# tahmidawal/Superresolution_for_PDEs

Hardware: AMD Instinct MI355X
Metric: 20->40 SR training samples/sec at batch 1024 per GPU (fwd+MSE bwd+clip+AdamW) (higher is better)
Workload: dtype f32 (h3: fp32 products from power-of-two-scaled 2-piece fp16 splits on fp16 MFMA, fp32 accumulate); 1 GPU; UNet 20->40 train step, fp32, batch 1024/GPU, 40x40; global_batch=1024, per_gpu_batch=1024, hw=40x40, parallelism=dp1

## Files before the change

superresolution_for_pdes_amd/csrc/conv.hip:

```cpp
#include "conv_common.h"

namespace srpde {



constexpr int BK = 16;
constexpr int LDK = BK + 4;


template <int BM, int BN, int WM, int WN>
__global__ __launch_bounds__(256) void conv_igemm_fwd_kernel(ConvParams p) {
  constexpr int TM = BM / WM, TN = BN / WN, TI = TM / 32, TJ = TN / 32;
  constexpr int A_LOADS = BM / 64;
  constexpr int B_ROWS_PER_PASS = 64;
  constexpr int B_LOADS = BN >= 64 ? BN / 64 : 1;
  extern __shared__ __attribute__((aligned(16))) float smem[];
  float* As = smem;
  float* Bs = smem + 2 * BM * LDK;

  const int tid = threadIdx.x, lane = tid & 63, wave = tid >> 6;
  const int wmi = wave % WM, wni = wave / WM;
  const int nbn = (p.Cout + BN - 1) / BN;
  const int nbm = (p.P + BM - 1) / BM;
  const int wg = xcd_remap(blockIdx.x, nbm * nbn);
// ... 758 lines not shown
    for (int g = 0; g < GA; ++g) {
      const unsigned off = (pok && a_ok[g]) ? (unsigned)(pix * p.lddy * 4 + a_colb[g]) : OOB;
      dma16(rsy, off, lds_addr_of(abase + g * GSTR));
    }
    char* bbase = abase + GA * GSTR;
#pragma unroll
    for (int g = 0; g < GB; ++g) {
      const int iy = yy + b_dy[g], ix = xx + b_dx[g];
      const bool ok = pok && b_ok[g] && iy >= 0 && iy < p.H && ix >= 0 && ix < p.W;
      const int ld = b_second[g] ? ld1 : p.ldx0;
      const unsigned off = ok ? (unsigned)((pix + b_sh[g]) * ld * 4 + b_chb[g]) : OOB;
      dma16(b_second[g] ? rs1 : rs0, off, lds_addr_of(bbase + g * GSTR));
    }
  };

  floatx16 acc[QA][QB], part[QA][QB];
#pragma unroll
  for (int i = 0; i < QA; ++i)
#pragma unroll
    for (int j = 0; j < QB; ++j)
#pragma unroll
      for (int r = 0; r < 16; ++r) acc[i][j][r] = 0.f;

  const int lr = lane & 31, lh = lane >> 5;
  const int wm0 = wmi * TM, wn0 = wni * TN;
  const int ma = wm0 + QA * lr, nb = wn0 + QB * lr;
  const int a_rd = (ma >> 5) * GSTR + (ma & 31) * 4 + lh * 128;
  const int b_rd = GA * GSTR + (nb >> 5) * GSTR + (nb & 31) * 4 + lh * 128;

  const int nsteps = (pend - pbeg + BKW - 1) / BKW;
  if (nsteps > 0) issue(pbeg, 0);
  asm volatile("s_waitcnt vmcnt(0)" ::: "memory");
  __syncthreads();
  for (int s = 0; s < nsteps; ++s) {
    const int buf = s & 1;
    if (s + 1 < nsteps) issue(pbeg + (s + 1) * BKW, buf ^ 1);
    const char* st = lds + buf * STAGE;
    const bool fresh = (s % HP) == 0;
#pragma unroll
    for (int kp = 0; kp < BKW / 2; ++kp) {
      const va_t av = *reinterpret_cast<const va_t*>(st + a_rd + kp * 256);
      const vb_t bv = *reinterpret_cast<const vb_t*>(st + b_rd + kp * 256);
#pragma unroll
      for (int i = 0; i < QA; ++i)
#pragma unroll
        for (int j = 0; j < QB; ++j) {
          const floatx16 c0 = (kp == 0 && fresh) ? floatx16{} : part[i][j];
          part[i][j] = __builtin_amdgcn_mfma_f32_32x32x2f32(vget(av, i), vget(bv, j), c0, 0, 0, 0);
        }
    }
    if ((s + 1) % HP == 0 || s + 1 == nsteps) {
#pragma unroll
      for (int i = 0; i < QA; ++i)
#pragma unroll
        for (int j = 0; j < QB; ++j) acc[i][j] += part[i][j];
    }
    asm volatile("s_waitcnt vmcnt(0)" ::: "memory");
    __syncthreads();
  }

  float* out = p.part + (size_t)split * p.Cout * p.K;
  const int n = n0 + nb;
  if (n < p.K) {
#pragma unroll
    for (int i = 0; i < QA; ++i)
#pragma unroll
      for (int r = 0; r < 16; ++r) {
        const int rc = (r & 3) + 8 * (r >> 2) + 4 * lh;
        const int m = m0 + wm0 + QA * rc + i;
        if (m < p.Cout) {
          float* dst = out + (size_t)m * p.K + n;
          if constexpr (QB == 1) {
            dst[0] = acc[i][0][r];
          } else if constexpr (QB == 2) {
            *reinterpret_cast<float2*>(dst) = make_float2(acc[i][0][r], acc[i][1][r]);
          } else {
            *reinterpret_cast<float4*>(dst) = make_float4(acc[i][0][r], acc[i][1][r], acc[i][2][r], acc[i][3][r]);
          }
        }
      }
  }
}

template <int G>
__global__ void slab_group_sum_kernel(float* __restrict__ part, int splits, long long total) {
  const long long i = (long long)blockIdx.x * blockDim.x + threadIdx.x;
  const long long ngroups = (splits + G - 1) / G;
  if (i >= total * ngroups) return;
  const long long g = i / total, e = i - g * total;
  const int q0 = (int)(g * G), q1 = min(splits, q0 + G);
  float s = 0.f;
  if (q1 - q0 == G) {
    float v[G];
#pragma unroll
    for (int u = 0; u < G; ++u) v[u] = part[(size_t)(q0 + u) * total + e];
#pragma unroll
    for (int u = 0; u < G; ++u) s += v[u];
  } else {
    for (int q = q0; q < q1; ++q) s += part[(size_t)q * total + e];
  }
  part[(size_t)q0 * total + e] = s;
}

__global__ void wgrad_reduce_kernel(const float* __restrict__ part, float* __restrict__ dw, int splits,
                                    int cout, int cin, int cin_real, int taps, int accumulate, int stride) {
  __shared__ float red[4][64];
  const long long K = (long long)taps * cin;
  const long long total = (long long)cout * K;
  const int el = threadIdx.x & 63, grp = threadIdx.x >> 6;
  const long long e = (long long)blockIdx.x * 64 + el;
  float s = 0.f;
  if (e < total) {
    const size_t qs = (size_t)stride * cout * K;
    int q = grp;
    for (; q + 28 < splits; q += 32) {
      float v[8];
#pragma unroll
      for (int u = 0; u < 8; ++u) v[u] = part[(size_t)(q + 4 * u) * qs + e];
#pragma unroll
      for (int u = 0; u < 8; ++u) s += v[u];
    }
    for (; q < splits; q += 4) s += part[(size_t)q * qs + e];
  }
  red[grp][el] = s;
  __syncthreads();
  if (grp == 0 && e < total) {
    const float v = (red[0][el] + red[1][el]) + (red[2][el] + red[3][el]);
    const int n = (int)(e / K);
    const int k = (int)(e - (long long)n * K);
    const int t = k / cin, c = k - t * cin;
    if (c < cin_real) {
      const long long dst = ((long long)n * cin_real + c) * taps + t;
      dw[dst] = accumulate ? dw[dst] + v : v;
    }
  }
}

int wgrad_reduce(const float* part, float* dw, int splits, int cout, int cin, int cin_real, int taps, int accumulate,
                 hipStream_t stream) {
  const long long total = (long long)cout * taps * cin;
  const int blocks = (int)((total + 63) / 64);
  int stride = 1;
  if (total < 65536 && splits >= 128) {
    constexpr int G = 32;
    const long long work = total * ((splits + G - 1) / G);
    hipLaunchKernelGGL(slab_group_sum_kernel<G>, dim3((int)((work + 255) / 256)), dim3(256), 0, stream,
                       const_cast<float*>(part), splits, total);
    SRPDE_LAUNCH_CHECK("srpde_conv_wgrad(reduce groups)");
    stride = G;
    splits = (splits + G - 1) / G;
  }
  hipLaunchKernelGGL(wgrad_reduce_kernel, dim3(blocks), dim3(256), 0, stream, part, dw, splits, cout, cin, cin_real,
                     taps, accumulate, stride);
  SRPDE_LAUNCH_CHECK("srpde_conv_wgrad(reduce)");
  return 0;
}

__global__ void pack_weights_kernel(const float* __restrict__ w, float* __restrict__ wf, float* __restrict__ wd,
                                    int cout, int cin, int cin_real, int taps) {
  const long long total = (long long)cout * taps * cin;
  for (long long e = blockIdx.x * (long long)blockDim.x + threadIdx.x; e < total;
       e += (long long)gridDim.x * blockDim.x) {
    const int c = (int)(e % cin);
    const long long r = e / cin;
    const int t = (int)(r % taps);
    const int n = (int)(r / taps);
    const float v = c < cin_real ? w[((long long)n * cin_real + c) * taps + t] : 0.f;
    if (wf) wf[e] = v;
    if (wd) wd[((long long)c * taps + t) * cout + n] = v;
  }
}

template <int BM, int BN, int WM, int WN>
static int launch_fwd(const ConvParams& p, hipStream_t st) {
  const int nbm = ceil_div(p.P, BM), nbn = ceil_div(p.Cout, BN);
  const size_t lds = (size_t)2 * (BM + BN) * LDK * sizeof(float);
  hipLaunchKernelGGL((conv_igemm_fwd_kernel<BM, BN, WM, WN>), dim3(nbm * nbn), dim3(256), lds, st, p);
  SRPDE_LAUNCH_CHECK("srpde_conv_fwd");
  return 0;
}


template <int BM, int BN, int WM, int WN, int HP>
static int launch_fwd_v2(ConvParams p, hipStream_t st, void* ws, size_t ws_bytes) {
  const int nbm = ceil_div(p.P, BM), nbn = ceil_div(p.Cout, BN);
  const int T = nbm * nbn;
  const size_t lds = (size_t)2 * (BM + BN) * ROW2;
  static int slots = [&] {
    int per_cu = 0, dev = 0, cus = 0;
    (void)hipGetDevice(&dev);
    (void)hipDeviceGetAttribute(&cus, hipDeviceAttributeMultiprocessorCount, dev);
    (void)hipOccupancyMaxActiveBlocksPerMultiprocessor(&per_cu, conv_fwd_v2_kernel<BM, BN, WM, WN, HP>, 256, lds);
    return std::max(1, per_cu) * std::max(1, cus);
  }();
  plan_tail(p, T, slots, BM, BN, ws, ws_bytes);
  const int grid = T - p.ntail + p.ntail * p.tsplit;
  hipLaunchKernelGGL((conv_fwd_v2_kernel<BM, BN, WM, WN, HP>), dim3(grid), dim3(256), lds, st, p);
  SRPDE_LAUNCH_CHECK("srpde_conv_fwd(v2)");
  if (p.ntail > 0) {
    hipLaunchKernelGGL((conv_tail_fixup_kernel<BM, BN>), dim3(p.ntail), dim3(1024), 0, st, p);
    SRPDE_LAUNCH_CHECK("srpde_conv_fwd(tail fixup)");
  }
  return 0;
}


static bool v2_ok(const ConvParams& p) {
  const long long maxld = std::max(p.ldx0, p.c1 ? p.ldx1 : 0);
  return p.c0 % 32 == 0 && p.c1 % 32 == 0 && (long long)p.P * maxld * 4 < (1LL << 31) &&
         (long long)p.Cout * p.K * 4 < (1LL << 31);
}

static int fwd_config(int cout) { return cout % 128 == 0 ? 0 : (cout % 64 == 0 ? 1 : 2); }
static int fwd_bm(int cfg) { return cfg == 0 ? 128 : 256; }

template <int BM, int BN, int WM, int WN>
static int launch_wgrad(const WgradParams& p, hipStream_t st, const WgradBn* bn = nullptr) {
  const int nb = ceil_div(p.Cout, BM) * ceil_div(p.K, BN) * p.splits;
  const size_t lds = (size_t)2 * BKP * ((BM + 4) + (BN + 4)) * sizeof(float);
  if (bn != nullptr)
    hipLaunchKernelGGL((conv_wgrad_kernel<BM, BN, WM, WN, true>), dim3(nb), dim3(256), lds, st, p, *bn);
  else
    hipLaunchKernelGGL((conv_wgrad_kernel<BM, BN, WM, WN, false>), dim3(nb), dim3(256), lds, st, p, WgradBn{});
  SRPDE_LAUNCH_CHECK("srpde_conv_wgrad");
  return 0;
}

template <int BM, int BN, int WM, int WN>
static int launch_wgrad_v2(const WgradParams& p, hipStream_t st) {
  const int nb = ceil_div(p.Cout, BM) * ceil_div(p.K, BN) * p.splits;
  const size_t lds = (size_t)2 * (BM / 32 + BN / 32) * GSTR;
  hipLaunchKernelGGL((conv_wgrad_v2_kernel<BM, BN, WM, WN, 2>), dim3(nb), dim3(256), lds, st, p);
  SRPDE_LAUNCH_CHECK("srpde_conv_wgrad(v2)");
  return 0;
}

// ... 181 lines not shown
```

superresolution_for_pdes_amd/csrc/pointwise.hip:

```cpp
#include "common.h"
#include "resample.h"

namespace srpde {

__global__ void nchw_to_nhwc_kernel(const float* __restrict__ x, float* __restrict__ out, int N, int Cin, int HW,
                                    int Cpad) {
  const long long total = (long long)N * HW;
  for (long long e = blockIdx.x * (long long)blockDim.x + threadIdx.x; e < total;
       e += (long long)gridDim.x * blockDim.x) {
    const long long n = e / HW;
    const int p = (int)(e - n * HW);
    float* o = out + e * Cpad;
    for (int c = 0; c < Cpad; ++c) o[c] = c < Cin ? x[(n * Cin + c) * HW + p] : 0.f;
  }
}

__global__ void nhwc_to_nchw_kernel(const float* __restrict__ x, int ldx, float* __restrict__ out, int N, int C,
                                    int HW) {
  const long long total = (long long)N * C * HW;
  for (long long e = blockIdx.x * (long long)blockDim.x + threadIdx.x; e < total;
       e += (long long)gridDim.x * blockDim.x) {
    const long long nc = e / HW;
    const int p = (int)(e - nc * HW);
    const long long n = nc / C;
// ... 817 lines not shown
    const float4 g = *reinterpret_cast<const float4*>(dm + n * C + c);
    const float s = sa[p];
    float4 o;
    o.x = (d.x * s) * a.x + g.x; o.y = (d.y * s) * a.y + g.y;
    o.z = (d.z * s) * a.z + g.z; o.w = (d.w * s) * a.w + g.w;
    float* dst = dx + p * lddx + c;
    if (accumulate) {
      const float4 old = *reinterpret_cast<const float4*>(dst);
      o.x += old.x; o.y += old.y; o.z += old.z; o.w += old.w;
    }
    *reinterpret_cast<float4*>(dst) = o;
  }
}

__global__ void att_bwd_gating_kernel(const float* __restrict__ dsa_pre, const float* __restrict__ wg,
                                      float* __restrict__ dg, int lddg, long long P, int G, int accumulate) {
  const int G4 = G >> 2;
  const long long total = P * G4;
  for (long long e = blockIdx.x * (long long)blockDim.x + threadIdx.x; e < total;
       e += (long long)gridDim.x * blockDim.x) {
    const long long p = e / G4;
    const int c = (int)(e - p * G4) * 4;
    const float s = dsa_pre[p];
    const float4 w = *reinterpret_cast<const float4*>(wg + c);
    float4 o = make_float4(s * w.x, s * w.y, s * w.z, s * w.w);
    float* dst = dg + p * lddg + c;
    if (accumulate) {
      const float4 old = *reinterpret_cast<const float4*>(dst);
      o.x += old.x; o.y += old.y; o.z += old.z; o.w += old.w;
    }
    *reinterpret_cast<float4*>(dst) = o;
  }
}

__global__ __launch_bounds__(256) void weighted_colsum_kernel(const float* __restrict__ v, int ldv,
                                                              const float* __restrict__ s, long long P, int C,
                                                              int rows_per_blk, float2* __restrict__ part) {
  extern __shared__ float4 red4[];
  const int C4 = C >> 2;
  const int c4 = threadIdx.x % C4, r0 = threadIdx.x / C4, rs = blockDim.x / C4;
  const int active = C4 * rs;
  float4 acc = make_float4(0.f, 0.f, 0.f, 0.f);
  float sacc = 0.f;
  const long long pb = (long long)blockIdx.x * rows_per_blk;
  const long long pe = min(P, pb + rows_per_blk);
  if ((int)threadIdx.x < active) {
    auto row = [&](const float4& a, float w) {
      acc.x += a.x * w; acc.y += a.y * w; acc.z += a.z * w; acc.w += a.w * w;
      if (c4 == 0) sacc += w;
    };
    long long p = pb + r0;
    for (; p + 3 * rs < pe; p += 4 * rs) {
      float4 a[4];
      float w[4];
#pragma unroll
      for (int u = 0; u < 4; ++u) {
        a[u] = *reinterpret_cast<const float4*>(v + (p + u * rs) * ldv + c4 * 4);
        w[u] = s[p + u * rs];
      }
#pragma unroll
      for (int u = 0; u < 4; ++u) row(a[u], w[u]);
    }
    for (; p < pe; p += rs) row(*reinterpret_cast<const float4*>(v + p * ldv + c4 * 4), s[p]);
  }
  red4[threadIdx.x] = acc;
  red4[256 + threadIdx.x] = make_float4(sacc, 0.f, 0.f, 0.f);
  __syncthreads();
  if ((int)threadIdx.x < C4) {
    float4 t = make_float4(0.f, 0.f, 0.f, 0.f);
    float ts = 0.f;
    for (int r = 0; r < rs; ++r) {
      const float4 a = red4[r * C4 + threadIdx.x];
      t.x += a.x; t.y += a.y; t.z += a.z; t.w += a.w;
      if (threadIdx.x == 0) ts += red4[256 + r * C4].x;
    }
    float2* o = part + (size_t)blockIdx.x * (C + 1);
    const int c = threadIdx.x * 4;
    o[c] = make_float2(t.x, 0.f); o[c + 1] = make_float2(t.y, 0.f);
    o[c + 2] = make_float2(t.z, 0.f); o[c + 3] = make_float2(t.w, 0.f);
    if (threadIdx.x == 0) o[C] = make_float2(ts, 0.f);
  }
}

__global__ __launch_bounds__(1024) void outer_sum_kernel(const float* __restrict__ a, int la,
                                                         const float* __restrict__ b, int lb, int n,
                                                         float* __restrict__ out) {
  __shared__ double red[16][64];
  const int i = blockIdx.x, jl = threadIdx.x & 63, grp = threadIdx.x >> 6;
  const int j = blockIdx.y * 64 + jl;
  double s = 0.0;
  if (j < lb) {
    int k = grp;
    for (; k + 7 * 16 < n; k += 8 * 16) {
      float av[8], bv[8];
#pragma unroll
      for (int u = 0; u < 8; ++u) {
        av[u] = a ? a[(long long)(k + 16 * u) * la + i] : 1.f;
        bv[u] = b ? b[(long long)(k + 16 * u) * lb + j] : 1.f;
      }
#pragma unroll
      for (int u = 0; u < 8; ++u) s += (double)av[u] * (double)bv[u];
    }
    for (; k < n; k += 16) {
      const double av = a ? (double)a[(long long)k * la + i] : 1.0;
      const double bv = b ? (double)b[(long long)k * lb + j] : 1.0;
      s += av * bv;
    }
  }
  red[grp][jl] = s;
  __syncthreads();
  if (grp == 0 && j < lb) {
    double t = 0.0;
    for (int g = 0; g < 16; ++g) t += red[g][jl];
    out[(long long)i * lb + j] = (float)t;
  }
}

__global__ void rowsum_kernel(const float* __restrict__ rows, int n, int len, float* __restrict__ out, int stride_in,
                              int accumulate) {
  const int j = blockIdx.x * blockDim.x + threadIdx.x;
  if (j >= len) return;
  double s = 0.0;
  for (int k = 0; k < n; ++k) s += rows[(long long)k * stride_in + j];
  out[j] = accumulate ? out[j] + (float)s : (float)s;
}

__global__ void partsum_kernel(const float2* __restrict__ part, int nblk, int len, float* __restrict__ out) {
  const int j = blockIdx.x;
  __shared__ double a[256];
  double s = 0.0;
  for (int k = threadIdx.x; k < nblk; k += 256) s += part[(size_t)k * len + j].x;
  a[threadIdx.x] = s;
  __syncthreads();
  for (int t = 128; t > 0; t >>= 1) {
    if ((int)threadIdx.x < t) a[threadIdx.x] += a[threadIdx.x + t];
    __syncthreads();
  }
  if (threadIdx.x == 0) out[j] = (float)a[0];
}

__global__ void head_fwd_kernel(const float* __restrict__ z, int ldz, int C, const float* __restrict__ wf,
                                const float* __restrict__ bf, const float* __restrict__ xin, int xin_c, int HW,
                                long long P, float* __restrict__ out) {
  for (long long p = blockIdx.x * (long long)blockDim.x + threadIdx.x; p < P; p += (long long)gridDim.x * blockDim.x) {
    float acc = 0.f;
    for (int c = 0; c < C; c += 4) {
      const float4 v = *reinterpret_cast<const float4*>(z + p * ldz + c);
      acc += v.x * wf[c] + v.y * wf[c + 1] + v.z * wf[c + 2] + v.w * wf[c + 3];
    }
    const long long n = p / HW;
    const int q = (int)(p - n * HW);
    out[p] = (acc + bf[0]) + xin[(n * xin_c) * HW + q];
  }
}

__global__ void head_bwd_dz_kernel(const float* __restrict__ dout, const float* __restrict__ wf, int C,
                                   float* __restrict__ dz, int lddz, long long P) {
  const int C4 = C >> 2;
  const long long total = P * C4;
  for (long long e = blockIdx.x * (long long)blockDim.x + threadIdx.x; e < total;
       e += (long long)gridDim.x * blockDim.x) {
    const long long p = e / C4;
    const int c = (int)(e - p * C4) * 4;
    const float d = dout[p];
    *reinterpret_cast<float4*>(dz + p * lddz + c) = make_float4(d * wf[c], d * wf[c + 1], d * wf[c + 2], d * wf[c + 3]);
  }
}

__global__ __launch_bounds__(256) void mse_partial_kernel(const float* __restrict__ y, const float* __restrict__ t,
                                                          long long n, double* __restrict__ part) {
  __shared__ double red[256];
  double s = 0.0;
  for (long long i = blockIdx.x * (long long)blockDim.x + threadIdx.x; i < n; i += (long long)gridDim.x * blockDim.x) {
    const float d = y[i] - t[i];
    s += (double)(d * d);
  }
  red[threadIdx.x] = s;
  __syncthreads();
  for (int k = 128; k > 0; k >>= 1) {
    if ((int)threadIdx.x < k) red[threadIdx.x] += red[threadIdx.x + k];
    __syncthreads();
  }
  if (threadIdx.x == 0) part[blockIdx.x] = red[0];
}

__global__ void mse_final_kernel(const double* __restrict__ part, int nblk, long long n, float* __restrict__ loss) {
  __shared__ double red[256];
  double s = 0.0;
  for (int k = threadIdx.x; k < nblk; k += 256) s += part[k];
  red[threadIdx.x] = s;
  __syncthreads();
  for (int k = 128; k > 0; k >>= 1) {
    if ((int)threadIdx.x < k) red[threadIdx.x] += red[threadIdx.x + k];
    __syncthreads();
  }
  if (threadIdx.x == 0) loss[0] = (float)(red[0] / (double)n);
}

__global__ void mse_bwd_kernel(const float* __restrict__ y, const float* __restrict__ t, long long n,
                               const float* __restrict__ gout, float* __restrict__ dy) {
  const float g = gout ? gout[0] : 1.f;
  const float norm = 2.f / (float)n;
  for (long long i = blockIdx.x * (long long)blockDim.x + threadIdx.x; i < n; i += (long long)gridDim.x * blockDim.x)
    dy[i] = norm * (y[i] - t[i]) * g;
}

static int grid_for(long long total, int cap = 8192) {
  long long b = (total + 255) / 256;
  if (b < 1) b = 1;
  return (int)std::min<long long>(b, cap);
}

static int colsum_blocks(long long P, int C, int* rpb) {
  const int rs = 256 / (C >> 2);
  long long r = (P + 1023) / 1024;
  r = (r + rs - 1) / rs * rs;
  if (r < rs) r = rs;
  *rpb = (int)r;
  return (int)((P + r - 1) / r);
}

// ... 177 lines not shown
  SRPDE_LAUNCH_CHECK("srpde_upsample_bilinear_bwd_gated_bn");
  return 0;
}

int srpde_upsample_bilinear_bwd(const float* dout, int lddo, float* dx, int lddx, int n, int h, int w, int ho,
                                int wo, int c, int accumulate, hipStream_t stream) {
  SRPDE_CHECK_ARG(dout && dx && c % 4 == 0 && ho >= h && wo >= w, "srpde_upsample_bilinear_bwd: bad args");
  SRPDE_CHECK_ARG(upsample_gather_ok(h, ho) && upsample_gather_ok(w, wo),
                  "srpde_upsample_bilinear_bwd: upsampling ratio above 4 (%dx%d -> %dx%d)", h, w, ho, wo);
  if (upsample_rows_ok(h, w, ho, wo, c, lddo, lddx)) {
    launch_upsample_bwd_rows<false>(dout, lddo, dx, lddx, n, h, w, ho, wo, c, accumulate, nullptr, nullptr, stream);
    SRPDE_LAUNCH_CHECK("srpde_upsample_bilinear_bwd");
    return 0;
  }
  dim3 g, b;
  if (px_geometry((long long)n * h * w, c, &g, &b)) {
    hipLaunchKernelGGL(upsample_bwd_px_kernel, g, b, 0, stream, dout, lddo, dx, lddx, (unsigned)(n * h * w), h, w, ho,
                       wo, accumulate);
    SRPDE_LAUNCH_CHECK("srpde_upsample_bilinear_bwd");
    return 0;
  }
  hipLaunchKernelGGL(upsample_bwd_kernel, dim3(grid_for((long long)n * h * w * (c / 4))), dim3(256), 0, stream, dout,
                     lddo, dx, lddx, n, h, w, ho, wo, c, accumulate);
  SRPDE_LAUNCH_CHECK("srpde_upsample_bilinear_bwd");
  return 0;
}

int srpde_att_channel_fwd(const float* x, int ldx, int n, int hw, int c, const float* w1, const float* b1,
                          const float* w2, const float* b2, float* m, float* hbuf, float* ca, hipStream_t stream) {
  SRPDE_CHECK_ARG(x && w1 && b1 && w2 && b2 && m && hbuf && ca, "srpde_att_channel_fwd: null");
  SRPDE_CHECK_ARG(c % 32 == 0 && c <= 1024, "srpde_att_channel_fwd: channel count");
  const int cr = c / 8;
  const size_t lds = (4 * 256 + c + cr) * sizeof(float);
  hipLaunchKernelGGL(att_channel_fwd_kernel, dim3(n), dim3(256), lds, stream, x, ldx, hw, c, cr, w1, b1, w2, b2, m,
                     hbuf, ca);
  SRPDE_LAUNCH_CHECK("srpde_att_channel_fwd");
  return 0;
}

int srpde_att_gate_fwd(const float* x, int ldx, const float* g, int ldg, int n, int hw, int c, int gc,
                       const float* ca, const float* wg, const float* bg, float* sa, float* out, int ldo,
                       hipStream_t stream) {
  SRPDE_CHECK_ARG(x && g && ca && wg && bg && sa && out, "srpde_att_gate_fwd: null");
  SRPDE_CHECK_ARG(c % 32 == 0 && gc % 4 == 0 && c <= 1024, "srpde_att_gate_fwd: channel counts");
  const long long P = (long long)n * hw;
  hipLaunchKernelGGL(att_spatial_fwd_kernel, dim3(grid_for(P * 8)), dim3(256), 0, stream, g, ldg, P, gc, wg, bg, sa);
  SRPDE_LAUNCH_CHECK("srpde_att_gate_fwd(spatial)");
  hipLaunchKernelGGL(att_apply_kernel, dim3(grid_for(P * (c / 4))), dim3(256), 0, stream, x, ldx, ca, sa, out, ldo,
                     P, hw, c);
  SRPDE_LAUNCH_CHECK("srpde_att_gate_fwd(apply)");
  return 0;
}

int srpde_att_fwd(const float* x, int ldx, const float* g, int ldg, int n, int hw, int c, int gc, const float* w1,
                  const float* b1, const float* w2, const float* b2, const float* wg, const float* bg, float* m,
                  float* hbuf, float* ca, float* sa, float* out, int ldo, hipStream_t stream) {
  SRPDE_CHECK_ARG(x && g && w1 && b1 && w2 && b2 && wg && bg && m && hbuf && ca && sa && out,
                  "srpde_att_fwd: null");
  SRPDE_CHECK_ARG(c % 32 == 0 && gc % 4 == 0 && c <= 1024, "srpde_att_fwd: channel counts");
  const int cr = c / 8;
  const size_t lds = (4 * 256 + c + cr) * sizeof(float);
  hipLaunchKernelGGL(att_channel_fwd_kernel, dim3(n), dim3(256), lds, stream, x, ldx, hw, c, cr, w1, b1, w2, b2, m,
                     hbuf, ca);
  SRPDE_LAUNCH_CHECK("srpde_att_fwd(channel)");
  const long long P = (long long)n * hw;
  hipLaunchKernelGGL(att_spatial_fwd_kernel, dim3(grid_for(P * 8)), dim3(256), 0, stream, g, ldg, P, gc, wg, bg, sa);
  SRPDE_LAUNCH_CHECK("srpde_att_fwd(spatial)");
  hipLaunchKernelGGL(att_apply_kernel, dim3(grid_for(P * (c / 4))), dim3(256), 0, stream, x, ldx, ca, sa, out, ldo,
                     P, hw, c);
  SRPDE_LAUNCH_CHECK("srpde_att_fwd(apply)");
  return 0;
}

size_t srpde_att_bwd_workspace_size(int n, int hw, int c, int gc) {
  const long long P = (long long)n * hw;
  const int cr = c / 8;
  int rpb;
  const int nb = colsum_blocks(P, gc, &rpb);
  size_t f = (size_t)P
             + (size_t)n * c
             + (size_t)n * cr * c * 2
             + (size_t)n * (cr + c)
             + (size_t)nb * (gc + 1) * 2;
  return f * sizeof(float) + 256;
}

int srpde_att_bwd(const float* dout, int lddo, const float* x, int ldx, const float* g, int ldg, int n, int hw,
                  int c, int gc, const float* w1, const float* w2, const float* wg, const float* m, const float* hbuf,
                  const float* ca, const float* sa, float* dx, int lddx, int dx_accumulate, float* dg, int lddg,
                  int dg_accumulate, float* dw1, float* db1, float* dw2, float* db2, float* dwg, float* dbg,
                  void* workspace, size_t ws_bytes, hipStream_t stream) {
  SRPDE_CHECK_ARG(dout && x && g && workspace, "srpde_att_bwd: null");
  SRPDE_CHECK_ARG(c % 32 == 0 && gc % 4 == 0, "srpde_att_bwd: channel counts");
  if (ws_bytes < srpde_att_bwd_workspace_size(n, hw, c, gc)) {
    set_error("srpde_att_bwd: workspace too small");
    return kErrWorkspace;
  }
  const long long P = (long long)n * hw;
  const int cr = c / 8;
  float* dsa = static_cast<float*>(workspace);
  float* dm = dsa + P;
  float* dw1r = dm + (size_t)n * c;
  float* dw2r = dw1r + (size_t)n * cr * c;
  float* db1r = dw2r + (size_t)n * cr * c;
  float* db2r = db1r + (size_t)n * cr;
  float2* part = reinterpret_cast<float2*>(db2r + (size_t)n * c + 2);
  part = reinterpret_cast<float2*>((reinterpret_cast<uintptr_t>(part) + 15) & ~uintptr_t(15));

  const size_t lds = (4 * 256 + c + cr) * sizeof(float);
  if (c == 64 || c == 128 || c == 256) {
    hipLaunchKernelGGL(att_bwd_sample_kernel, dim3(n), dim3(256), lds, stream, dout, lddo, x, ldx, sa, hw, c, cr, w1,
                       w2, m, hbuf, ca, dm, dw1r, db1r, dw2r, db2r, dsa);
    SRPDE_LAUNCH_CHECK("srpde_att_bwd(sample)");
  } else {
    hipLaunchKernelGGL(att_bwd_pixel_kernel, dim3(grid_for(P * 8)), dim3(256), 0, stream, dout, lddo, x, ldx, ca,
                       sa, P, hw, c, dsa);
    SRPDE_LAUNCH_CHECK("srpde_att_bwd(pixel)");
    hipLaunchKernelGGL(att_bwd_channel_kernel, dim3(n), dim3(256), lds, stream, dout, lddo, x, ldx, sa, hw, c, cr,
                       w1, w2, m, hbuf, ca, dm, dw1r, db1r, dw2r, db2r);
    SRPDE_LAUNCH_CHECK("srpde_att_bwd(channel)");
  }
  if (dx != nullptr) {
    hipLaunchKernelGGL(att_bwd_dx_kernel, dim3(grid_for(P * (c / 4))), dim3(256), 0, stream, dout, lddo, ca, sa, dm,
                       dx, lddx, P, hw, c, dx_accumulate);
    SRPDE_LAUNCH_CHECK("srpde_att_bwd(dx)");
  }
  if (dg != nullptr) {
    hipLaunchKernelGGL(att_bwd_gating_kernel, dim3(grid_for(P * (gc / 4))), dim3(256), 0, stream, dsa, wg, dg, lddg,
                       P, gc, dg_accumulate);
    SRPDE_LAUNCH_CHECK("srpde_att_bwd(gating)");
  }
  if (dw1 == nullptr) return 0;
  return srpde_att_bwd_params(g, ldg, n, hw, c, gc, m, hbuf, dw1, db1, dw2, db2, dwg, dbg, workspace, ws_bytes,
                              stream);
}

__global__ __launch_bounds__(256) void upsample_t_scalar_kernel(const float* __restrict__ dsa, float* __restrict__ st,
                                                                int n, int h, int w, int ho, int wo) {
  const long long q = (long long)blockIdx.x * blockDim.x + threadIdx.x;
  if (q >= (long long)n * h * w) return;
  const int ix = (int)(q % w), iy = (int)((q / w) % h), nn = (int)(q / ((long long)w * h));
  int ylo, yhi, xlo, xhi;
  cand_range(iy, h, ho, &ylo, &yhi);
  cand_range(ix, w, wo, &xlo, &xhi);
  const float* base = dsa + (size_t)nn * ho * wo;
  float s = 0.f;
  for (int oy = ylo; oy <= yhi; ++oy) {
    bool hy;
    const float wy = cand_weight(oy, iy, h, ho, &hy);
    if (!hy) continue;
    float r = 0.f;
    for (int ox = xlo; ox <= xhi; ++ox) {
      bool hx;
      const float wx = cand_weight(ox, ix, w, wo, &hx);
      if (hx) r += wx * base[(size_t)oy * wo + ox];
    }
    s += wy * r;
  }
  st[q] = s;
}

static void att_params_outer(int n, int c, const float* m, const float* hbuf, const float* db1r, const float* db2r,
                             float* dw1, float* db1, float* dw2, float* db2, hipStream_t stream) {
  const int cr = c / 8;
  hipLaunchKernelGGL(outer_sum_kernel, dim3(cr, ceil_div(c, 64)), dim3(1024), 0, stream, db1r, cr, m, c, n, dw1);
  hipLaunchKernelGGL(outer_sum_kernel, dim3(c, ceil_div(cr, 64)), dim3(1024), 0, stream, db2r, c, hbuf, cr, n, dw2);
  hipLaunchKernelGGL(outer_sum_kernel, dim3(1, ceil_div(cr, 64)), dim3(1024), 0, stream, (const float*)nullptr, 1,
                     db1r, cr, n, db1);
  hipLaunchKernelGGL(outer_sum_kernel, dim3(1, ceil_div(c, 64)), dim3(1024), 0, stream, (const float*)nullptr, 1,
                     db2r, c, n, db2);
}

int srpde_att_bwd_params_lowres(const float* d, int ldd, int n, int h, int w, int ho, int wo, int c, int gc,
                                const float* m, const float* hbuf, float* dw1, float* db1, float* dw2, float* db2,
                                float* dwg, float* dbg, void* workspace, size_t ws_bytes, hipStream_t stream) {
  SRPDE_CHECK_ARG(d && m && hbuf && dw1 && db1 && dw2 && db2 && dwg && dbg && workspace && ldd % 4 == 0 && gc % 4 == 0 &&
                      c % 32 == 0 && ho >= h && wo >= w,
                  "srpde_att_bwd_params_lowres: bad args");
  const int hw = ho * wo;
  if (ws_bytes < srpde_att_bwd_workspace_size(n, hw, c, gc)) {
    set_error("srpde_att_bwd_params_lowres: workspace too small");
    return kErrWorkspace;
  }
  const long long P = (long long)n * hw, Plo = (long long)n * h * w;
  const int cr = c / 8;
  float* dsa = static_cast<float*>(workspace);
  float* dm = dsa + P;
  float* dw1r = dm + (size_t)n * c;
  float* dw2r = dw1r + (size_t)n * cr * c;
  float* db1r = dw2r + (size_t)n * cr * c;
  float* db2r = db1r + (size_t)n * cr;
  float2* part = reinterpret_cast<float2*>(db2r + (size_t)n * c + 2);
  part = reinterpret_cast<float2*>((reinterpret_cast<uintptr_t>(part) + 15) & ~uintptr_t(15));
  SRPDE_CHECK_ARG(Plo <= 2LL * n * cr * c, "srpde_att_bwd_params_lowres: low-res field larger than its scratch");
  float* st = dw1r;
  att_params_outer(n, c, m, hbuf, db1r, db2r, dw1, db1, dw2, db2, stream);
  SRPDE_LAUNCH_CHECK("srpde_att_bwd_params_lowres(rowsum)");
  hipLaunchKernelGGL(upsample_t_scalar_kernel, dim3((unsigned)((Plo + 255) / 256)), dim3(256), 0, stream, dsa, st, n, h,
                     w, ho, wo);
  SRPDE_LAUNCH_CHECK("srpde_att_bwd_params_lowres(transpose)");
  int rpb;
  const int nb = colsum_blocks(Plo, gc, &rpb);
  hipLaunchKernelGGL(weighted_colsum_kernel, dim3(nb), dim3(256), 2 * 256 * sizeof(float4), stream, d, ldd, st, Plo,
                     gc, rpb, part);
  SRPDE_LAUNCH_CHECK("srpde_att_bwd_params_lowres(colsum)");
  hipLaunchKernelGGL(partsum_kernel, dim3(gc), dim3(256), 0, stream, part, nb, gc + 1, dwg);
  hipLaunchKernelGGL(partsum_kernel, dim3(1), dim3(256), 0, stream, part + gc, nb, gc + 1, dbg);
  SRPDE_LAUNCH_CHECK("srpde_att_bwd_params_lowres(partsum)");
  return 0;
}

int srpde_att_bwd_params(const float* g, int ldg, int n, int hw, int c, int gc, const float* m, const float* hbuf,
                         float* dw1, float* db1, float* dw2, float* db2, float* dwg, float* dbg, void* workspace,
                         size_t ws_bytes, hipStream_t stream) {
  SRPDE_CHECK_ARG(g && m && hbuf && dw1 && db1 && dw2 && db2 && dwg && dbg && workspace,
                  "srpde_att_bwd_params: null");
  if (ws_bytes < srpde_att_bwd_workspace_size(n, hw, c, gc)) {
    set_error("srpde_att_bwd_params: workspace too small");
    return kErrWorkspace;
  }
  const long long P = (long long)n * hw;
  const int cr = c / 8;
  float* dsa = static_cast<float*>(workspace);
  float* dm = dsa + P;
  float* dw1r = dm + (size_t)n * c;
  float* dw2r = dw1r + (size_t)n * cr * c;
  float* db1r = dw2r + (size_t)n * cr * c;
  float* db2r = db1r + (size_t)n * cr;
  float2* part = reinterpret_cast<float2*>(db2r + (size_t)n * c + 2);
  part = reinterpret_cast<float2*>((reinterpret_cast<uintptr_t>(part) + 15) & ~uintptr_t(15));
  (void)dw1r; (void)dw2r; (void)cr;
  att_params_outer(n, c, m, hbuf, db1r, db2r, dw1, db1, dw2, db2, stream);
  SRPDE_LAUNCH_CHECK("srpde_att_bwd(rowsum)");
  int rpb;
  const int nb = colsum_blocks(P, gc, &rpb);
  hipLaunchKernelGGL(weighted_colsum_kernel, dim3(nb), dim3(256), 2 * 256 * sizeof(float4), stream, g, ldg, dsa, P,
                     gc, rpb, part);
  SRPDE_LAUNCH_CHECK("srpde_att_bwd(colsum)");
  hipLaunchKernelGGL(partsum_kernel, dim3(gc), dim3(256), 0, stream, part, nb, gc + 1, dwg);
  hipLaunchKernelGGL(partsum_kernel, dim3(1), dim3(256), 0, stream, part + gc, nb, gc + 1, dbg);
  SRPDE_LAUNCH_CHECK("srpde_att_bwd(partsum)");
  return 0;
}

int srpde_head_fwd(const float* z, int ldz, int c, const float* wf, const float* bf, const float* xin, int xin_c,
                   int n, int hw, float* out, hipStream_t stream) {
  SRPDE_CHECK_ARG(z && wf && bf && xin && out && c % 4 == 0, "srpde_head_fwd: bad args");
  const long long P = (long long)n * hw;
  hipLaunchKernelGGL(head_fwd_kernel, dim3(grid_for(P)), dim3(256), 0, stream, z, ldz, c, wf, bf, xin, xin_c, hw, P,
                     out);
  SRPDE_LAUNCH_CHECK("srpde_head_fwd");
  return 0;
}

size_t srpde_head_bwd_workspace_size(int n, int hw, int c) {
  int rpb;
  const int nb = colsum_blocks((long long)n * hw, c, &rpb);
  return (size_t)nb * (c + 1) * sizeof(float2);
}

int srpde_head_bwd(const float* dout, const float* z, int ldz, int c, const float* wf, int n, int hw, float* dz,
                   int lddz, float* dwf, float* dbf, void* workspace, size_t ws_bytes, hipStream_t stream) {
  SRPDE_CHECK_ARG(dout && z && wf && dz && dwf && dbf && workspace && c % 4 == 0, "srpde_head_bwd: bad args");
  if (ws_bytes < srpde_head_bwd_workspace_size(n, hw, c)) {
    set_error("srpde_head_bwd: workspace too small");
    return kErrWorkspace;
  }
  const long long P = (long long)n * hw;
  hipLaunchKernelGGL(head_bwd_dz_kernel, dim3(grid_for(P * (c / 4))), dim3(256), 0, stream, dout, wf, c, dz, lddz, P);
  SRPDE_LAUNCH_CHECK("srpde_head_bwd(dz)");
  int rpb;
  const int nb = colsum_blocks(P, c, &rpb);
  float2* part = static_cast<float2*>(workspace);
  hipLaunchKernelGGL(weighted_colsum_kernel, dim3(nb), dim3(256), 2 * 256 * sizeof(float4), stream, z, ldz, dout, P,
                     c, rpb, part);
  hipLaunchKernelGGL(partsum_kernel, dim3(c), dim3(256), 0, stream, part, nb, c + 1, dwf);
  hipLaunchKernelGGL(partsum_kernel, dim3(1), dim3(256), 0, stream, part + c, nb, c + 1, dbf);
  SRPDE_LAUNCH_CHECK("srpde_head_bwd(reduce)");
  return 0;
}

size_t srpde_mse_workspace_size(void) { return 1024 * sizeof(double); }

int srpde_mse_fwd(const float* y, const float* t, long long n, float* loss, void* workspace, size_t ws_bytes,
                  hipStream_t stream) {
  SRPDE_CHECK_ARG(y && t && loss && workspace && ws_bytes >= 1024 * sizeof(double), "srpde_mse_fwd: bad args");
  const int nb = (int)std::min<long long>(1024, std::max<long long>(1, (n + 255) / 256));
  hipLaunchKernelGGL(mse_partial_kernel, dim3(nb), dim3(256), 0, stream, y, t, n, static_cast<double*>(workspace));
  hipLaunchKernelGGL(mse_final_kernel, dim3(1), dim3(256), 0, stream, static_cast<const double*>(workspace), nb, n,
                     loss);
  SRPDE_LAUNCH_CHECK("srpde_mse_fwd");
  return 0;
}

int srpde_mse_bwd(const float* y, const float* t, long long n, const float* gout, float* dy, hipStream_t stream) {
  SRPDE_CHECK_ARG(y && t && dy, "srpde_mse_bwd: bad args");
  hipLaunchKernelGGL(mse_bwd_kernel, dim3(grid_for(n)), dim3(256), 0, stream, y, t, n, gout, dy);
  SRPDE_LAUNCH_CHECK("srpde_mse_bwd");
  return 0;
}

}
```

Before: 36610 samples/s.

## Vectorize wgrad reduction, tile attention MLP param grads, merge partsum launches

The weight-gradient split reduction now uses float4 loads and picks its group count and unroll depth from the split count. The attention MLP parameter gradients (dw1, dw2, db1, db2) were four strided outer-sum kernels; they become one LDS-tiled partial kernel over sample slices plus one combine kernel, with scratch placed in existing workspace. The two partsum launches for weight and bias are merged into one launch. These target memory throughput and launch count in backward reductions, at the cost of extra template instances and more complex scratch layout.

```diff
diff --git a/superresolution_for_pdes_amd/csrc/conv.hip b/superresolution_for_pdes_amd/csrc/conv.hip
--- a/superresolution_for_pdes_amd/csrc/conv.hip
+++ b/superresolution_for_pdes_amd/csrc/conv.hip
@@ -864,52 +864,91 @@
   }
 }
 
-template <int G>
-__global__ void slab_group_sum_kernel(float* __restrict__ part, int splits, long long total) {
+template <int V>
+struct SlabVec;
+template <>
+struct SlabVec<1> {
+  float v[1];
+  __device__ void load(const float* p) { v[0] = *p; }
+  __device__ void store(float* p) const { *p = v[0]; }
+};
+template <>
+struct SlabVec<4> {
+  float v[4];
+  __device__ void load(const float* p) {
+    const float4 t = *reinterpret_cast<const float4*>(p);
+    v[0] = t.x; v[1] = t.y; v[2] = t.z; v[3] = t.w;
+  }
+  __device__ void store(float* p) const { *reinterpret_cast<float4*>(p) = make_float4(v[0], v[1], v[2], v[3]); }
+};
+
+template <int G, int V>
+__global__ __launch_bounds__(64) void slab_group_sum_kernel(float* __restrict__ part, int splits, long long total) {
   const long long i = (long long)blockIdx.x * blockDim.x + threadIdx.x;
-  const long long ngroups = (splits + G - 1) / G;
-  if (i >= total * ngroups) return;
-  const long long g = i / total, e = i - g * total;
+  const long long ngroups = (splits + G - 1) / G, tv = total / V;
+  if (i >= tv * ngroups) return;
+  const long long g = i / tv, e = (i - g * tv) * V;
   const int q0 = (int)(g * G), q1 = min(splits, q0 + G);
-  float s = 0.f;
+  SlabVec<V> s;
+#pragma unroll
+  for (int j = 0; j < V; ++j) s.v[j] = 0.f;
   if (q1 - q0 == G) {
-    float v[G];
-#pragma unroll
-    for (int u = 0; u < G; ++u) v[u] = part[(size_t)(q0 + u) * total + e];
-#pragma unroll
-    for (int u = 0; u < G; ++u) s += v[u];
+    SlabVec<V> v[G];
+#pragma unroll
+    for (int u = 0; u < G; ++u) v[u].load(part + (size_t)(q0 + u) * total + e);
+#pragma unroll
+    for (int u = 0; u < G; ++u)
+#pragma unroll
+      for (int j = 0; j < V; ++j) s.v[j] += v[u].v[j];
   } else {
-    for (int q = q0; q < q1; ++q) s += part[(size_t)q * total + e];
-  }
-  part[(size_t)q0 * total + e] = s;
-}
-
-__global__ void wgrad_reduce_kernel(const float* __restrict__ part, float* __restrict__ dw, int splits,
-                                    int cout, int cin, int cin_real, int taps, int accumulate, int stride) {
-  __shared__ float red[4][64];
+    for (int q = q0; q < q1; ++q) {
+      SlabVec<V> v;
+      v.load(part + (size_t)q * total + e);
+#pragma unroll
+      for (int j = 0; j < V; ++j) s.v[j] += v.v[j];
+    }
+  }
+  s.store(part + (size_t)q0 * total + e);
+}
+
+template <int V, int GR, int NB>
+__global__ __launch_bounds__(256) void wgrad_reduce_kernel(const float* __restrict__ part, float* __restrict__ dw,
+                                                           int splits, int cout, int cin, int cin_real, int taps,
+                                                           int accumulate, int stride) {
+  constexpr int EL = 256 / GR, BE = EL * V;
+  __shared__ float red[GR][BE];
   const long long K = (long long)taps * cin;
   const long long total = (long long)cout * K;
-  const int el = threadIdx.x & 63, grp = threadIdx.x >> 6;
-  const long long e = (long long)blockIdx.x * 64 + el;
-  float s = 0.f;
+  const int el = threadIdx.x % EL, grp = threadIdx.x / EL;
+  const long long e = (long long)blockIdx.x * BE + el * V;
+  float s[V];
+#pragma unroll
+  for (int j = 0; j < V; ++j) s[j] = 0.f;
   if (e < total) {
     const size_t qs = (size_t)stride * cout * K;
-    int q = grp;
-    for (; q + 28 < splits; q += 32) {
-      float v[8];
-#pragma unroll
-      for (int u = 0; u < 8; ++u) v[u] = part[(size_t)(q + 4 * u) * qs + e];
-#pragma unroll
-      for (int u = 0; u < 8; ++u) s += v[u];
-    }
-    for (; q < splits; q += 4) s += part[(size_t)q * qs + e];
-  }
-  red[grp][el] = s;
+    for (int q = grp; q < splits; q += GR * NB) {
+      SlabVec<V> v[NB];
+#pragma unroll
+      for (int u = 0; u < NB; ++u)
+        if (q + GR * u < splits) v[u].load(part + (size_t)(q + GR * u) * qs + e);
+#pragma unroll
+      for (int u = 0; u < NB; ++u)
+        if (q + GR * u < splits) {
+#pragma unroll
+          for (int j = 0; j < V; ++j) s[j] += v[u].v[j];
+        }
+    }
+  }
+#pragma unroll
+  for (int j = 0; j < V; ++j) red[grp][el * V + j] = s[j];
   __syncthreads();
-  if (grp == 0 && e < total) {
-    const float v = (red[0][el] + red[1][el]) + (red[2][el] + red[3][el]);
-    const int n = (int)(e / K);
-    const int k = (int)(e - (long long)n * K);
+  const long long eo = (long long)blockIdx.x * BE + threadIdx.x;
+  if ((int)threadIdx.x < BE && eo < total) {
+    float v = red[0][threadIdx.x];
+#pragma unroll
+    for (int g = 1; g < GR; ++g) v += red[g][threadIdx.x];
+    const int n = (int)(eo / K);
+    const int k = (int)(eo - (long long)n * K);
     const int t = k / cin, c = k - t * cin;
     if (c < cin_real) {
       const long long dst = ((long long)n * cin_real + c) * taps + t;
@@ -918,22 +957,36 @@
   }
 }
 
+template <int V>
+static void launch_wgrad_reduce(const float* part, float* dw, int splits, int cout, int cin, int cin_real, int taps,
+                                int accumulate, long long total, hipStream_t stream) {
+  int stride = 1;
+  const bool few = total < 65536;
+  if (few && splits >= 128) {
+    constexpr int G = 32;
+    const long long work = total / V * ((splits + G - 1) / G);
+    hipLaunchKernelGGL((slab_group_sum_kernel<G, V>), dim3((unsigned)((work + 63) / 64)), dim3(64), 0, stream,
+                       const_cast<float*>(part), splits, total);
+    stride = G;
+    splits = (splits + G - 1) / G;
+  }
+  auto go = [&](auto kern, int be) {
+    hipLaunchKernelGGL(kern, dim3((unsigned)((total + be - 1) / be)), dim3(256), 0, stream, part, dw, splits, cout, cin,
+                       cin_real, taps, accumulate, stride);
+  };
+  if (few) go(wgrad_reduce_kernel<V, 32, 4>, 8 * V);
+  else if (splits <= 8) go(wgrad_reduce_kernel<V, 4, 2>, 64 * V);
+  else if (splits <= 16) go(wgrad_reduce_kernel<V, 4, 4>, 64 * V);
+  else go(wgrad_reduce_kernel<V, 4, 8>, 64 * V);
+}
+
 int wgrad_reduce(const float* part, float* dw, int splits, int cout, int cin, int cin_real, int taps, int accumulate,
                  hipStream_t stream) {
   const long long total = (long long)cout * taps * cin;
-  const int blocks = (int)((total + 63) / 64);
-  int stride = 1;
-  if (total < 65536 && splits >= 128) {
-    constexpr int G = 32;
-    const long long work = total * ((splits + G - 1) / G);
-    hipLaunchKernelGGL(slab_group_sum_kernel<G>, dim3((int)((work + 255) / 256)), dim3(256), 0, stream,
-                       const_cast<float*>(part), splits, total);
-    SRPDE_LAUNCH_CHECK("srpde_conv_wgrad(reduce groups)");
-    stride = G;
-    splits = (splits + G - 1) / G;
-  }
-  hipLaunchKernelGGL(wgrad_reduce_kernel, dim3(blocks), dim3(256), 0, stream, part, dw, splits, cout, cin, cin_real,
-                     taps, accumulate, stride);
+  if (total % 4 == 0 && aligned16(part))
+    launch_wgrad_reduce<4>(part, dw, splits, cout, cin, cin_real, taps, accumulate, total, stream);
+  else
+    launch_wgrad_reduce<1>(part, dw, splits, cout, cin, cin_real, taps, accumulate, total, stream);
   SRPDE_LAUNCH_CHECK("srpde_conv_wgrad(reduce)");
   return 0;
 }
diff --git a/superresolution_for_pdes_amd/csrc/pointwise.hip b/superresolution_for_pdes_amd/csrc/pointwise.hip
--- a/superresolution_for_pdes_amd/csrc/pointwise.hip
+++ b/superresolution_for_pdes_amd/csrc/pointwise.hip
@@ -923,37 +923,122 @@
   }
 }
 
-__global__ __launch_bounds__(1024) void outer_sum_kernel(const float* __restrict__ a, int la,
-                                                         const float* __restrict__ b, int lb, int n,
-                                                         float* __restrict__ out) {
-  __shared__ double red[16][64];
-  const int i = blockIdx.x, jl = threadIdx.x & 63, grp = threadIdx.x >> 6;
-  const int j = blockIdx.y * 64 + jl;
+constexpr int MLP_TC = 32, MLP_SPS_MIN = 4, MLP_SPS_MAX = 32;
+
+static long long att_mlp_rowlen(int c) { return 2LL * (c / 8) * c + c / 8 + c; }
+
+static int att_mlp_slices(int n, int c, int* sps) {
+  const int tiles = c / MLP_TC;
+  const int want = std::max(1, ceil_div(256, tiles));
+  *sps = std::min(MLP_SPS_MAX, std::max(MLP_SPS_MIN, ceil_div(n, want)));
+  return ceil_div(n, *sps);
+}
+
+static size_t att_mlp_scratch_floats(int n, int c) {
+  int sps;
+  return (size_t)att_mlp_slices(n, c, &sps) * att_mlp_rowlen(c) * 2 + 4;
+}
+
+template <bool VEC>
+__global__ __launch_bounds__(256) void att_mlp_partial_kernel(const float* __restrict__ db1r,
+                                                              const float* __restrict__ m,
+                                                              const float* __restrict__ db2r,
+                                                              const float* __restrict__ hbuf, int n, int C, int Cr,
+                                                              int sps, double* __restrict__ part) {
+  extern __shared__ float sh[];
+  float* s_dh = sh;
+  float* s_h = s_dh + sps * Cr;
+  float* s_m = s_h + sps * Cr;
+  float* s_dp = s_m + sps * MLP_TC;
+  const int k0 = blockIdx.x * sps, c0 = blockIdx.y * MLP_TC;
+  const int ns = min(sps, n - k0);
+  const int tid = threadIdx.x;
+  {
+    const float* gdh = db1r + (size_t)k0 * Cr;
+    const float* gh = hbuf + (size_t)k0 * Cr;
+    const float* gm = m + (size_t)k0 * C + c0;
+    const float* gdp = db2r + (size_t)k0 * C + c0;
+    if constexpr (VEC) {
+      for (int i = tid; i < ns * Cr / 4; i += 256) {
+        reinterpret_cast<float4*>(s_dh)[i] = reinterpret_cast<const float4*>(gdh)[i];
+        reinterpret_cast<float4*>(s_h)[i] = reinterpret_cast<const float4*>(gh)[i];
+      }
+      for (int i = tid; i < ns * (MLP_TC / 4); i += 256) {
+        const int k = i / (MLP_TC / 4), j = i % (MLP_TC / 4);
+        reinterpret_cast<float4*>(s_m)[i] = *reinterpret_cast<const float4*>(gm + (size_t)k * C + 4 * j);
+        reinterpret_cast<float4*>(s_dp)[i] = *reinterpret_cast<const float4*>(gdp + (size_t)k * C + 4 * j);
+      }
+    } else {
+      for (int i = tid; i < ns * Cr; i += 256) {
+        s_dh[i] = gdh[i];
+        s_h[i] = gh[i];
+      }
+      for (int i = tid; i < ns * MLP_TC; i += 256) {
+        const int k = i / MLP_TC, j = i % MLP_TC;
+        s_m[i] = gm[(size_t)k * C + j];
+        s_dp[i] = gdp[(size_t)k * C + j];
+      }
+    }
+  }
+  __syncthreads();
+  const long long w = (long long)Cr * C;
+  double* row = part + (size_t)blockIdx.x * (2 * w + Cr + C);
+  const int half = MLP_TC * Cr;
+  for (int o = tid; o < 2 * half; o += 256) {
+    double s = 0.0;
+    if (o < half) {
+      const int r = o / MLP_TC, cl = o % MLP_TC;
+      for (int k = 0; k < ns; ++k) s += (double)s_dh[k * Cr + r] * (double)s_m[k * MLP_TC + cl];
+      row[(long long)r * C + c0 + cl] = s;
+    } else {
+      const int cl = (o - half) / Cr, r = (o - half) % Cr;
+      for (int k = 0; k < ns; ++k) s += (double)s_dp[k * MLP_TC + cl] * (double)s_h[k * Cr + r];
+      row[w + (long long)(c0 + cl) * Cr + r] = s;
+    }
+  }
+  if (tid < MLP_TC) {
+    double s = 0.0;
+    for (int k = 0; k < ns; ++k) s += (double)s_dp[k * MLP_TC + tid];
+    row[2 * w + Cr + c0 + tid] = s;
+  }
+  if (blockIdx.y == 0)
+    for (int r = tid; r < Cr; r += 256) {
+      double s = 0.0;
+      for (int k = 0; k < ns; ++k) s += (double)s_dh[k * Cr + r];
+      row[2 * w + r] = s;
+    }
+}
+
+__global__ __launch_bounds__(256) void att_mlp_combine_kernel(const double* __restrict__ part, int slices, int C,
+                                                              int Cr, float* __restrict__ dw1,
+                                                              float* __restrict__ db1, float* __restrict__ dw2,
+                                                              float* __restrict__ db2) {
+  __shared__ double red[8][32];
+  const long long w = (long long)Cr * C, len = 2 * w + Cr + C;
+  const int el = threadIdx.x & 31, grp = threadIdx.x >> 5;
+  const long long j = (long long)blockIdx.x * 32 + el;
   double s = 0.0;
-  if (j < lb) {
+  if (j < len) {
     int k = grp;
-    for (; k + 7 * 16 < n; k += 8 * 16) {
-      float av[8], bv[8];
-#pragma unroll
-      for (int u = 0; u < 8; ++u) {
-        av[u] = a ? a[(long long)(k + 16 * u) * la + i] : 1.f;
-        bv[u] = b ? b[(long long)(k + 16 * u) * lb + j] : 1.f;
-      }
-#pragma unroll
-      for (int u = 0; u < 8; ++u) s += (double)av[u] * (double)bv[u];
-    }
-    for (; k < n; k += 16) {
-      const double av = a ? (double)a[(long long)k * la + i] : 1.0;
-      const double bv = b ? (double)b[(long long)k * lb + j] : 1.0;
-      s += av * bv;
-    }
-  }
-  red[grp][jl] = s;
+    for (; k + 3 * 8 < slices; k += 4 * 8) {
+      double v[4];
+#pragma unroll
+      for (int u = 0; u < 4; ++u) v[u] = part[(size_t)(k + 8 * u) * len + j];
+#pragma unroll
+      for (int u = 0; u < 4; ++u) s += v[u];
+    }
+    for (; k < slices; k += 8) s += part[(size_t)k * len + j];
+  }
+  red[grp][el] = s;
   __syncthreads();
-  if (grp == 0 && j < lb) {
+  if (grp == 0 && j < len) {
     double t = 0.0;
-    for (int g = 0; g < 16; ++g) t += red[g][jl];
-    out[(long long)i * lb + j] = (float)t;
+    for (int g = 0; g < 8; ++g) t += red[g][el];
+    const float v = (float)t;
+    if (j < w) dw1[j] = v;
+    else if (j < 2 * w) dw2[j - w] = v;
+    else if (j < 2 * w + Cr) db1[j - 2 * w] = v;
+    else db2[j - 2 * w - Cr] = v;
   }
 }
 
@@ -966,7 +1051,8 @@
   out[j] = accumulate ? out[j] + (float)s : (float)s;
 }
 
-__global__ void partsum_kernel(const float2* __restrict__ part, int nblk, int len, float* __restrict__ out) {
+__global__ void partsum_kernel(const float2* __restrict__ part, int nblk, int len, float* __restrict__ out, int split,
+                               float* __restrict__ out2) {
   const int j = blockIdx.x;
   __shared__ double a[256];
   double s = 0.0;
@@ -977,7 +1063,10 @@
     if ((int)threadIdx.x < t) a[threadIdx.x] += a[threadIdx.x + t];
     __syncthreads();
   }
-  if (threadIdx.x == 0) out[j] = (float)a[0];
+  if (threadIdx.x == 0) {
+    if (j < split) out[j] = (float)a[0];
+    else out2[j - split] = (float)a[0];
+  }
 }
 
 __global__ void head_fwd_kernel(const float* __restrict__ z, int ldz, int C, const float* __restrict__ wf,
@@ -1321,6 +1410,7 @@
              + (size_t)n * cr * c * 2
              + (size_t)n * (cr + c)
              + (size_t)nb * (gc + 1) * 2;
+  if (att_mlp_scratch_floats(n, c) > (size_t)n * cr * c * 2) f += att_mlp_scratch_floats(n, c) + 4;
   return f * sizeof(float) + 256;
 }
 
@@ -1400,14 +1490,24 @@
 }
 
 static void att_params_outer(int n, int c, const float* m, const float* hbuf, const float* db1r, const float* db2r,
-                             float* dw1, float* db1, float* dw2, float* db2, hipStream_t stream) {
+                             float* rows, const void* tail, float* dw1, float* db1, float* dw2, float* db2,
+                             hipStream_t stream) {
   const int cr = c / 8;
-  hipLaunchKernelGGL(outer_sum_kernel, dim3(cr, ceil_div(c, 64)), dim3(1024), 0, stream, db1r, cr, m, c, n, dw1);
-  hipLaunchKernelGGL(outer_sum_kernel, dim3(c, ceil_div(cr, 64)), dim3(1024), 0, stream, db2r, c, hbuf, cr, n, dw2);
-  hipLaunchKernelGGL(outer_sum_kernel, dim3(1, ceil_div(cr, 64)), dim3(1024), 0, stream, (const float*)nullptr, 1,
-                     db1r, cr, n, db1);
-  hipLaunchKernelGGL(outer_sum_kernel, dim3(1, ceil_div(c, 64)), dim3(1024), 0, stream, (const float*)nullptr, 1,
-                     db2r, c, n, db2);
+  int sps;
+  const int slices = att_mlp_slices(n, c, &sps);
+  const bool fits = att_mlp_scratch_floats(n, c) <= (size_t)n * cr * c * 2;
+  const uintptr_t at = fits ? reinterpret_cast<uintptr_t>(rows) : reinterpret_cast<uintptr_t>(tail);
+  double* part = reinterpret_cast<double*>((at + 15) & ~uintptr_t(15));
+  const size_t lds = (size_t)sps * (2 * cr + 2 * MLP_TC) * sizeof(float);
+  const dim3 grid(slices, c / MLP_TC);
+  if (aligned16(db1r) && aligned16(db2r) && aligned16(m) && aligned16(hbuf))
+    hipLaunchKernelGGL(att_mlp_partial_kernel<true>, grid, dim3(256), lds, stream, db1r, m, db2r, hbuf, n, c, cr, sps,
+                       part);
+  else
+    hipLaunchKernelGGL(att_mlp_partial_kernel<false>, grid, dim3(256), lds, stream, db1r, m, db2r, hbuf, n, c, cr, sps,
+                       part);
+  hipLaunchKernelGGL(att_mlp_combine_kernel, dim3((unsigned)ceil_div(att_mlp_rowlen(c), 32LL)), dim3(256), 0, stream,
+                     part, slices, c, cr, dw1, db1, dw2, db2);
 }
 
 int srpde_att_bwd_params_lowres(const float* d, int ldd, int n, int h, int w, int ho, int wo, int c, int gc,
@@ -1432,8 +1532,10 @@
   float2* part = reinterpret_cast<float2*>(db2r + (size_t)n * c + 2);
   part = reinterpret_cast<float2*>((reinterpret_cast<uintptr_t>(part) + 15) & ~uintptr_t(15));
   SRPDE_CHECK_ARG(Plo <= 2LL * n * cr * c, "srpde_att_bwd_params_lowres: low-res field larger than its scratch");
+  int rpb_full;
+  const void* tail = part + (size_t)colsum_blocks(P, gc, &rpb_full) * (gc + 1);
   float* st = dw1r;
-  att_params_outer(n, c, m, hbuf, db1r, db2r, dw1, db1, dw2, db2, stream);
+  att_params_outer(n, c, m, hbuf, db1r, db2r, dw1r, tail, dw1, db1, dw2, db2, stream);
   SRPDE_LAUNCH_CHECK("srpde_att_bwd_params_lowres(rowsum)");
   hipLaunchKernelGGL(upsample_t_scalar_kernel, dim3((unsigned)((Plo + 255) / 256)), dim3(256), 0, stream, dsa, st, n, h,
                      w, ho, wo);
@@ -1443,8 +1545,7 @@
   hipLaunchKernelGGL(weighted_colsum_kernel, dim3(nb), dim3(256), 2 * 256 * sizeof(float4), stream, d, ldd, st, Plo,
                      gc, rpb, part);
   SRPDE_LAUNCH_CHECK("srpde_att_bwd_params_lowres(colsum)");
-  hipLaunchKernelGGL(partsum_kernel, dim3(gc), dim3(256), 0, stream, part, nb, gc + 1, dwg);
-  hipLaunchKernelGGL(partsum_kernel, dim3(1), dim3(256), 0, stream, part + gc, nb, gc + 1, dbg);
+  hipLaunchKernelGGL(partsum_kernel, dim3(gc + 1), dim3(256), 0, stream, part, nb, gc + 1, dwg, gc, dbg);
   SRPDE_LAUNCH_CHECK("srpde_att_bwd_params_lowres(partsum)");
   return 0;
 }
@@ -1468,16 +1569,14 @@
   float* db2r = db1r + (size_t)n * cr;
   float2* part = reinterpret_cast<float2*>(db2r + (size_t)n * c + 2);
   part = reinterpret_cast<float2*>((reinterpret_cast<uintptr_t>(part) + 15) & ~uintptr_t(15));
-  (void)dw1r; (void)dw2r; (void)cr;
-  att_params_outer(n, c, m, hbuf, db1r, db2r, dw1, db1, dw2, db2, stream);
-  SRPDE_LAUNCH_CHECK("srpde_att_bwd(rowsum)");
   int rpb;
   const int nb = colsum_blocks(P, gc, &rpb);
+  att_params_outer(n, c, m, hbuf, db1r, db2r, dw1r, part + (size_t)nb * (gc + 1), dw1, db1, dw2, db2, stream);
+  SRPDE_LAUNCH_CHECK("srpde_att_bwd(rowsum)");
   hipLaunchKernelGGL(weighted_colsum_kernel, dim3(nb), dim3(256), 2 * 256 * sizeof(float4), stream, g, ldg, dsa, P,
                      gc, rpb, part);
   SRPDE_LAUNCH_CHECK("srpde_att_bwd(colsum)");
-  hipLaunchKernelGGL(partsum_kernel, dim3(gc), dim3(256), 0, stream, part, nb, gc + 1, dwg);
-  hipLaunchKernelGGL(partsum_kernel, dim3(1), dim3(256), 0, stream, part + gc, nb, gc + 1, dbg);
+  hipLaunchKernelGGL(partsum_kernel, dim3(gc + 1), dim3(256), 0, stream, part, nb, gc + 1, dwg, gc, dbg);
   SRPDE_LAUNCH_CHECK("srpde_att_bwd(partsum)");
   return 0;
 }
@@ -1513,8 +1612,7 @@
   float2* part = static_cast<float2*>(workspace);
   hipLaunchKernelGGL(weighted_colsum_kernel, dim3(nb), dim3(256), 2 * 256 * sizeof(float4), stream, z, ldz, dout, P,
                      c, rpb, part);
-  hipLaunchKernelGGL(partsum_kernel, dim3(c), dim3(256), 0, stream, part, nb, c + 1, dwf);
-  hipLaunchKernelGGL(partsum_kernel, dim3(1), dim3(256), 0, stream, part + c, nb, c + 1, dbf);
+  hipLaunchKernelGGL(partsum_kernel, dim3(c + 1), dim3(256), 0, stream, part, nb, c + 1, dwf, c, dbf);
   SRPDE_LAUNCH_CHECK("srpde_head_bwd(reduce)");
   return 0;
 }
```

Measured after the change: 36720 samples/s (median of 6 runs). No clear change (+0.3%).
